# TritonDataCenter/registrar

Hardware: NVIDIA H100
Metric: service-records/sec (higher is better)
Workload: dtype u8

## Files before the change

### registrar_b200/csrc/regk_api.cu

```cuda
#include <cuda_runtime.h>

#include <algorithm>
#include <cstdarg>
#include <cstdio>
#include <cstdlib>
#include <cstring>
#include <map>
#include <mutex>
#include <string>
#include <vector>

#include "../../include/regk.h"
#include "regk_kernels.cuh"
#include "regk_gather.cuh"
#include "regk_peersync.cuh"
#include "regk_service.cuh"
#include "regk_jute.cuh"
#include "regk_decode.cuh"
#include "regk_parents.cuh"
#include "regk_skip.cuh"
#include "regk_mkdirp.cuh"
#include "regk_types.hpp"

using namespace regk;

namespace {

thread_local std::string g_create_error;

struct DevBuf {
    void *p = nullptr;
    size_t cap = 0;
};

struct HostBuf {
    void *p = nullptr;
    size_t cap = 0;
};

}

struct regk_ctx {
    int device = 0;
    cudaStream_t own_stream = nullptr;
    cudaStream_t stream = nullptr;
    std::string err;
    int sm_count = 0;
    int max_smem_optin = 0;

    std::vector<std::string> types;
    std::vector<uint8_t> blob_host;
    DevBuf blob_dev;
    uint32_t max_type_q = 0;

    DevBuf in[11];
    DevBuf path_bytes, path_off, json_bytes, json_off, off32_p, off32_j;
    HostBuf h_path_bytes, h_path_off, h_json_bytes, h_json_off, h_running;
    cudaStream_t s_h2d = nullptr, s_d2h = nullptr;
    struct HostSet {
        DevBuf in[11];
        DevBuf path_bytes, path_off, json_bytes, json_off, off32_p, off32_j;
        HostBuf h_path_bytes, h_path_off, h_json_bytes, h_json_off;
        cudaEvent_t e_in = nullptr, e_out = nullptr;
    };
    HostSet hset[2];
    uint64_t hseq = 0;
    uint32_t *h_gather_flag = nullptr;
    double json_mean_seen = 0.0;
    uint64_t json_est_seen = 0;
    bool json_learning = true;
    regk_job job{};
    bool job_bound = false;
    unsigned long long job_seq = 0;
    DevBuf job_bases;
    unsigned long long *h_job_bases = nullptr;
    const uint8_t *last_path_bytes = nullptr;
    const unsigned long long *last_path_off = nullptr;
    uint64_t last_n = 0;
    const uint8_t *last_json_bytes = nullptr;
    const unsigned long long *last_json_off = nullptr;
    uint64_t last_json_n = 0;
    DevBuf jute_bytes, jute_off;
    HostBuf h_jute_bytes, h_jute_off;
    DevBuf dec_in[4], dec_rec, dec_dom, dec_ports;
    HostBuf h_dec_rec, h_dec_dom, h_dec_ports;
    const uint32_t *last_host_off = nullptr;
    uint32_t last_host_stride = 0;
    bool last_alias = false;
    DevBuf svc_in[7], svc_work;
    DevBuf par_len, par_slot, par_table, par_totals, par_unique;
    cudaEvent_t par_ev[2] = {nullptr, nullptr};
    HostBuf h_par_len, h_par_unique, h_par_count;
    enum { MK_PLEN, MK_PSLOT, MK_PTABLE, MK_PTOTALS, MK_PUNIQUE, MK_FLAGS, MK_LIST0, MK_LIST1, MK_TOTALS, MK_TABLE,
           MK_COUNT, MK_DREC, MK_DLEN, MK_DBYTES, MK_DOFF, MK_DEPTH, MK_INVALID, MK_ZERO, MK_FBYTES, MK_FOFF, MK_NBUF };
    DevBuf mk[MK_NBUF];
    HostBuf h_mk_count, h_mk_drec, h_mk_dlen, h_mk_dbytes, h_mk_doff, h_mk_depth, h_mk_invalid, h_mk_fbytes, h_mk_foff;
    cudaEvent_t mk_ev[4] = {nullptr, nullptr, nullptr, nullptr};
    bool mk_valid = false;
    uint64_t mk_n_dirs = 0, mk_bytes = 0;
    std::vector<cudaEvent_t> pipe_events;
    DevBuf skip_work, skip_in[11], skip_off_p, skip_off_j, skip_index, skip_bits;
    HostBuf h_skip_status, h_skip_index, h_skip_bits;
    struct SkipLast {
        bool valid = false;
        uint64_t n = 0, n_skipped = 0;
        uint32_t bad_bits = 0;
    } skip_last;
    DevBuf work;
    static constexpr int NWORK = 4;
    DevBuf work_ring[NWORK];
    cudaEvent_t ws_clean[NWORK] = {nullptr, nullptr, nullptr, nullptr};
    size_t ws_clean_bytes[NWORK] = {0, 0, 0, 0};
    cudaStream_t s_side = nullptr;
    uint64_t ws_seq = 0;

    struct Slot {
        cudaEvent_t ev[6] = {nullptr, nullptr, nullptr, nullptr, nullptr, nullptr};
        PathParams path_params{};
        size_t path_smem = 0;
        bool path_alias = false, did_path = false;
        DevStatus *d_status = nullptr;
        DevStatus *h_status = nullptr;
        int ring = -1;
        int hset = -1;
        bool d2h_issued = false;
        bool timed = true;
        const uint8_t *dev_path_bytes = nullptr;
        const unsigned long long *dev_path_off = nullptr;
        const uint8_t *dev_json_bytes = nullptr;
        const unsigned long long *dev_json_off = nullptr;
        const uint32_t *dev_host_off = nullptr;
// ... 23 lines not shown
namespace {

int fail(regk_ctx *c, int code, const char *fmt, ...)
{
    char buf[512];
    va_list ap;
    va_start(ap, fmt);
    vsnprintf(buf, sizeof buf, fmt, ap);
    va_end(ap);
    if (c)
        c->err = buf;
    else
        g_create_error = buf;
    return code;
}

#define CK(call)                                                                                   \
    do {                                                                                           \
        cudaError_t e_ = (call);                                                                   \
        if (e_ != cudaSuccess)                                                                     \
            return fail(ctx, REGK_ERR_CUDA, "%s failed: %s (%s:%d)", #call, cudaGetErrorString(e_), \
                __FILE__, __LINE__);                                                               \
    } while (0)

int ensure_dev(regk_ctx *ctx, DevBuf &b, size_t bytes)
{
    bytes = (bytes + 255) & ~(size_t)255;
    if (bytes <= b.cap)
        return REGK_OK;
    if (b.p)
        CK(cudaFree(b.p));
    b.p = nullptr;
    b.cap = 0;
    size_t want = bytes + bytes / 8;
    cudaError_t e = cudaMalloc(&b.p, want);
    if (e != cudaSuccess) {
        cudaGetLastError();
        e = cudaMalloc(&b.p, bytes);
        want = bytes;
    }
    if (e != cudaSuccess)
        return fail(ctx, REGK_ERR_NOMEM, "cudaMalloc(%zu) failed: %s", bytes, cudaGetErrorString(e));
    b.cap = want;
    return REGK_OK;
}

int ensure_host(regk_ctx *ctx, HostBuf &b, size_t bytes)
{
    bytes = (bytes + 4095) & ~(size_t)4095;
    if (bytes <= b.cap)
        return REGK_OK;
    if (b.p)
        CK(cudaFreeHost(b.p));
    b.p = nullptr;
    b.cap = 0;
    cudaError_t e = cudaMallocHost(&b.p, bytes);
    if (e != cudaSuccess)
        return fail(ctx, REGK_ERR_NOMEM, "cudaMallocHost(%zu) failed: %s", bytes, cudaGetErrorString(e));
    b.cap = bytes;
    return REGK_OK;
}

int64_t opt_get(const regk_ctx *c, const char *name, int64_t dflt)
{
    auto it = c->opt.find(name);
    return it == c->opt.end() ? dflt : it->second;
}

size_t align16(size_t v)
{
    return (v + 15) & ~(size_t)15;
}

bool smem_attr_needs_raise(int device, int which, size_t bytes)
{
    static std::mutex mu;
    static size_t high[64][4];
    std::lock_guard<std::mutex> lock(mu);
    size_t &h = high[device & 63][which];
    if (bytes <= h)
        return false;
    h = bytes;
    return true;
}

}

__global__ void __launch_bounds__(256) regk_off32_kernel(const unsigned long long *__restrict__ src, uint32_t *__restrict__ dst, uint64_t n1)
{
    const uint64_t i = (uint64_t)blockIdx.x * 256 + threadIdx.x;
    if (i < n1)
        dst[i] = (uint32_t)src[i];
}

static int narrow_offsets(regk_ctx *ctx, const void *src64, DevBuf &dst32, uint64_t n, cudaStream_t s)
{
    int rc = ensure_dev(ctx, dst32, (n + 1) * 4);
    if (rc)
        return rc;
    regk_off32_kernel<<<(unsigned)((n + 1 + 255) / 256), 256, 0, s>>>((const unsigned long long *)src64, (uint32_t *)dst32.p, n + 1);
    CK(cudaGetLastError());
    return REGK_OK;
}

struct HostPipe {
    uint64_t chunk = 0, nchunks = 0, nsuper_chunk = 0;
    unsigned long long *running = nullptr;
    uint64_t path_cap = 0, json_cap = 0;
    const void *src[11] = {};
    void *dev[11] = {};
};

static bool chunk_bounds_ok(const regk_batch *b, uint64_t chunk, bool do_path, bool do_json, bool alias)
{
    const uint64_t n = b->n;
    auto ok = [&](const uint32_t *off) {
        if (!off)
            return true;
        uint32_t prev = off[0];
        const uint32_t last = off[n];
        if (prev != 0 && prev > last)
            return false;
        for (uint64_t r = chunk; r < n; r += chunk) {
            if (off[r] < prev || off[r] > last)
                return false;
            prev = off[r];
        }
        return true;
    };
    return (!do_path || (ok(b->domain_off) && (alias || ok(b->host_off)))) &&
           (!do_json || (ok(b->addr_off) && ok(b->ports_off)));
}

static int run_pipelined(regk_ctx *ctx, const regk_batch *b, regk_result *res, const PathParams &pp0, size_t path_smem,
    const JsonParams &jp0, size_t json_smem, const HostPipe &hp)
{
    const uint64_t n = b->n;
    const bool alias = b->flags & REGK_NODE_ALIAS;
    const bool do_path = !(b->flags & REGK_NO_PATH), do_json = !(b->flags & REGK_NO_JSON);
    const uint32_t stride = b->host_stride;
    cudaStream_t s = ctx->stream;
    int rc;
    if (!ctx->s_h2d) {
        CK(cudaStreamCreateWithFlags(&ctx->s_h2d, cudaStreamNonBlocking));
        CK(cudaStreamCreateWithFlags(&ctx->s_d2h, cudaStreamNonBlocking));
    }
    while (ctx->pipe_events.size() < 3 * hp.nchunks + 2) {
        cudaEvent_t e;
        CK(cudaEventCreateWithFlags(&e, cudaEventDisableTiming));
        ctx->pipe_events.push_back(e);
    }
    if ((rc = ensure_host(ctx, ctx->h_path_bytes, hp.path_cap)) || (rc = ensure_host(ctx, ctx->h_path_off, (n + 1) * 8)) ||
        (rc = ensure_host(ctx, ctx->h_json_bytes, hp.json_cap)) || (rc = ensure_host(ctx, ctx->h_json_off, (n + 1) * 8)) ||
        (rc = ensure_host(ctx, ctx->h_running, (hp.nchunks + 2) * 8)))
        return rc;
    unsigned long long *h_running = (unsigned long long *)ctx->h_running.p;
    DevStatus *d_status = pp0.status ? pp0.status : jp0.status;
    DevStatus *h_status = ctx->slots[0].h_status;

    cudaEvent_t e_ready = ctx->pipe_events[3 * hp.nchunks];
    CK(cudaEventRecord(e_ready, s));
    CK(cudaStreamWaitEvent(ctx->s_h2d, e_ready, 0));

    const uint32_t *dom_off = (const uint32_t *)b->domain_off, *host_off = (const uint32_t *)b->host_off,
                   *addr_off = (const uint32_t *)b->addr_off, *ports_off = (const uint32_t *)b->ports_off;
    auto h2d = [&](int i, size_t byte_lo, size_t byte_hi) -> cudaError_t {
// ... 560 lines not shown
    CK(cudaSetDevice(ctx->device));
    std::vector<std::string> raw(ntypes);
    for (uint32_t i = 0; i < ntypes; i++)
        raw[i].assign(types[i], lens ? lens[i] : strlen(types[i]));
    std::vector<uint8_t> blob;
    uint32_t maxq = 0;
    std::string why;
    const int brc = build_type_blob(raw, &blob, &maxq, &why);
    if (brc)
        return fail(ctx, brc == 1 ? REGK_ERR_OUT_OF_DOMAIN : REGK_ERR_INVALID_ARG, "regk_set_types: %s", why.c_str());
    int rc = ensure_dev(ctx, ctx->blob_dev, blob.size());
    if (rc)
        return rc;
    CK(cudaMemcpyAsync(ctx->blob_dev.p, blob.data(), blob.size(), cudaMemcpyHostToDevice, ctx->stream));
    CK(cudaStreamSynchronize(ctx->stream));
    ctx->types = raw;
    ctx->blob_host = blob;
    ctx->max_type_q = maxq;
    ctx->json_mean_seen = 0.0;
    ctx->json_learning = true;
    return REGK_OK;
}

void *regk_host_alloc(regk_ctx *ctx, size_t bytes)
{
    if (!ctx)
        return nullptr;
    void *p = nullptr;
    cudaSetDevice(ctx->device);
    if (cudaMallocHost(&p, bytes ? bytes : 1) != cudaSuccess) {
        cudaGetLastError();
        return nullptr;
    }
    return p;
}

void regk_host_free(regk_ctx *ctx, void *p)
{
    (void)ctx;
    if (p)
        cudaFreeHost(p);
}

void *regk_dev_alloc(regk_ctx *ctx, size_t bytes)
{
    if (!ctx)
        return nullptr;
    void *p = nullptr;
    cudaSetDevice(ctx->device);
    if (cudaMalloc(&p, bytes ? bytes : 1) != cudaSuccess) {
        cudaGetLastError();
        return nullptr;
    }
    return p;
}

void regk_dev_free(regk_ctx *ctx, void *p)
{
    (void)ctx;
    if (p)
        cudaFree(p);
}

int regk_memcpy_h2d(regk_ctx *ctx, void *dst_dev, const void *src_host, size_t bytes)
{
    if (!ctx)
        return REGK_ERR_INVALID_ARG;
    CK(cudaSetDevice(ctx->device));
    CK(cudaMemcpyAsync(dst_dev, src_host, bytes, cudaMemcpyHostToDevice, ctx->stream));
    CK(cudaStreamSynchronize(ctx->stream));
    return REGK_OK;
}

int regk_memcpy_d2h(regk_ctx *ctx, void *dst_host, const void *src_dev, size_t bytes)
{
    if (!ctx)
        return REGK_ERR_INVALID_ARG;
    CK(cudaSetDevice(ctx->device));
    CK(cudaMemcpyAsync(dst_host, src_dev, bytes, cudaMemcpyDeviceToHost, ctx->stream));
    CK(cudaStreamSynchronize(ctx->stream));
    return REGK_OK;
}

int regk_sync(regk_ctx *ctx)
{
    if (!ctx)
        return REGK_ERR_INVALID_ARG;
    CK(cudaSetDevice(ctx->device));
    CK(cudaStreamSynchronize(ctx->stream));
    if (ctx->h_gather_flag && *ctx->h_gather_flag) {
        *ctx->h_gather_flag = 0;
        return fail(ctx, REGK_ERR_INVALID_ARG, "regk_gather_push: the totals table exceeds the whole-job buffers or disagrees with the shard; nothing was stored");
    }
    return REGK_OK;
}

int regk_ipc_export(regk_ctx *ctx, const void *dev_ptr, unsigned char handle[REGK_IPC_HANDLE_BYTES])
{
    if (!ctx || !dev_ptr || !handle)
        return fail(ctx, REGK_ERR_INVALID_ARG, "regk_ipc_export: NULL argument");
    static_assert(sizeof(cudaIpcMemHandle_t) == REGK_IPC_HANDLE_BYTES, "IPC handle size");
    CK(cudaSetDevice(ctx->device));
    cudaIpcMemHandle_t h;
    CK(cudaIpcGetMemHandle(&h, const_cast<void *>(dev_ptr)));
    memcpy(handle, &h, sizeof h);
    return REGK_OK;
}

int regk_ipc_open(regk_ctx *ctx, const unsigned char handle[REGK_IPC_HANDLE_BYTES], void **peer_ptr)
{
    if (!ctx || !handle || !peer_ptr)
        return fail(ctx, REGK_ERR_INVALID_ARG, "regk_ipc_open: NULL argument");
    CK(cudaSetDevice(ctx->device));
    cudaIpcMemHandle_t h;
    memcpy(&h, handle, sizeof h);
    *peer_ptr = nullptr;
    CK(cudaIpcOpenMemHandle(peer_ptr, h, cudaIpcMemLazyEnablePeerAccess));
    return REGK_OK;
}

int regk_ipc_close(regk_ctx *ctx, void *peer_ptr)
{
    if (!ctx || !peer_ptr)
        return REGK_ERR_INVALID_ARG;
    CK(cudaSetDevice(ctx->device));
    CK(cudaIpcCloseMemHandle(peer_ptr));
    return REGK_OK;
}

int regk_gather_push(regk_ctx *ctx, const regk_result *shard, const regk_gather *g)
{
    if (!ctx || !shard || !g)
        return fail(ctx, REGK_ERR_INVALID_ARG, "regk_gather_push: NULL argument");
    if (g->world == 0 || g->world > REGK_MAX_PEERS || g->rank >= g->world)
        return fail(ctx, REGK_ERR_INVALID_ARG, "regk_gather_push: world %u / rank %u out of range (at most %d peers)",
            g->world, g->rank, REGK_MAX_PEERS);
    if (!(shard->flags & REGK_OUT_DEVICE) || !shard->path_off || !shard->json_off)
        return fail(ctx, REGK_ERR_INVALID_ARG, "regk_gather_push: the shard must be a finished REGK_OUT_DEVICE result");
    if (!g->totals || g->rec_base + shard->n > g->n_total)
        return fail(ctx, REGK_ERR_INVALID_ARG, "regk_gather_push: totals missing or record range outside the job");
    for (uint32_t q = 0; q < g->world; q++)
        if (!g->path_bytes[q] || !g->path_off[q] || !g->json_bytes[q] || !g->json_off[q] ||
            (((uintptr_t)g->path_bytes[q] | (uintptr_t)g->json_bytes[q]) & 15) || (((uintptr_t)g->path_off[q] | (uintptr_t)g->json_off[q]) & 7))
            return fail(ctx, REGK_ERR_INVALID_ARG, "regk_gather_push: buffer of rank %u missing or misaligned", q);
    CK(cudaSetDevice(ctx->device));
    if (!ctx->h_gather_flag) {
        CK(cudaMallocHost((void **)&ctx->h_gather_flag, sizeof(uint32_t)));
        *ctx->h_gather_flag = 0;
    }
    GatherParams p{};
    p.world = g->world;
    p.rank = g->rank;
    p.n_local = shard->n;
    p.rec_base = g->rec_base;
    p.n_total = g->n_total;
    p.totals = (const unsigned long long *)g->totals;
    p.src_path = shard->path_bytes;
    p.src_json = shard->json_bytes;
    p.src_path_off = (const unsigned long long *)shard->path_off;
    p.src_json_off = (const unsigned long long *)shard->json_off;
    for (uint32_t q = 0; q < g->world; q++) {
        p.dst_path[q] = (uint8_t *)g->path_bytes[q];
        p.dst_json[q] = (uint8_t *)g->json_bytes[q];
        p.dst_path_off[q] = (unsigned long long *)g->path_off[q];
        p.dst_json_off[q] = (unsigned long long *)g->json_off[q];
    }
// ... 230 lines not shown
        wk = (uint8_t *)ctx->work.p;
        CK(cudaMemsetAsync(wk, 0, work_bytes, s));
    } else {
        ring = (int)(ctx->ws_seq++ % regk_ctx::NWORK);
        if (!ctx->s_side) {
            CK(cudaStreamCreateWithFlags(&ctx->s_side, cudaStreamNonBlocking));
            for (auto &e : ctx->ws_clean)
                CK(cudaEventCreateWithFlags(&e, cudaEventDisableTiming));
        }
        const size_t cap_before = ctx->work_ring[ring].cap;
        if ((rc = ensure_dev(ctx, ctx->work_ring[ring], work_bytes)))
            return rc;
        if (ctx->work_ring[ring].cap != cap_before)
            ctx->ws_clean_bytes[ring] = 0;
        wk = (uint8_t *)ctx->work_ring[ring].p;
        if (ctx->ws_clean_bytes[ring] >= work_bytes)
        {
            if (cudaEventQuery(ctx->ws_clean[ring]) != cudaSuccess) {
                cudaGetLastError();
                CK(cudaStreamWaitEvent(s, ctx->ws_clean[ring], 0));
            }
        }
        else
            CK(cudaMemsetAsync(wk, 0, work_bytes, s));
    }
    DevStatus *d_status = (DevStatus *)wk;

    if (n == 0 && !job) {
        CK(cudaMemsetAsync(o_path_off.p, 0, 8, s));
        CK(cudaMemsetAsync(o_json_off.p, 0, 8, s));
    }
    const uint32_t force_generic = (uint32_t)opt_get(ctx, "force_generic", 0);

    PathParams pp{};
    size_t path_smem = 0;
    if (n && do_path) {
        pp.n = n;
        pp.domain_bytes = (const uint8_t *)dev[0];
        pp.domain_off = (const uint32_t *)dev[1];
        pp.host_bytes = (const uint8_t *)dev[2];
        pp.host_off = (const uint32_t *)dev[3];
        pp.host_stride = b->host_stride;
        pp.out_bytes = out_path_bytes;
        pp.out_off = out_path_off;
        pp.out_capacity = out_path_cap;
        if (job) {
            pp.bias_in = d_bases;
            fill_peers(pp.peer, J, J.path_bytes, J.path_off);
        }
        pp.exact = 0;
        pp.tile_total = (uint32_t *)(wk + totals_p_off);
        pp.super_total = (unsigned long long *)(wk + super_p_off);
        pp.status = d_status;
        pp.dom_limit = dom_len;
        pp.host_limit = host_len;
        pp.force_generic = force_generic;
        const uint64_t mean_dom_tile = std::min<uint64_t>(dom_len, dom_len * TILE / std::max<uint64_t>(n, 1)) + 1;
        uint32_t dom_cap = (uint32_t)opt_get(ctx, "dom_cap", 0);
        if (!dom_cap)
            dom_cap = (uint32_t)std::min<uint64_t>(std::max<uint64_t>(align16(mean_dom_tile * 5 / 4 + 384), 2048), 49152);
        dom_cap = (uint32_t)((dom_cap + 127) & ~127u);
        uint32_t host_cap = 0;
        if (!alias) {
            const uint64_t mean_host_tile = pp.host_off ? std::min<uint64_t>(host_len, host_len * TILE / std::max<uint64_t>(n, 1)) + 1
                                                        : (uint64_t)TILE * b->host_stride;
            host_cap = (uint32_t)std::min<uint64_t>(align16((pp.host_off ? mean_host_tile * 3 / 2 + 512 : mean_host_tile) + 16), 49152);
        }
        const uint32_t out_cap = (uint32_t)align16((uint64_t)dom_cap + host_cap + 2 * TILE + 32);
        path_smem = 16 + (size_t)dom_cap + 32 + dom_cap / 8 + 16 + (alias ? 0 : host_cap + 32) + out_cap + 32;
        if (path_smem > (size_t)ctx->max_smem_optin)
            return fail(ctx, REGK_ERR_INVALID_ARG, "path kernel needs %zu B of shared memory (> %d)", path_smem, ctx->max_smem_optin);
        pp.dom_cap = dom_cap;
        pp.host_cap = host_cap;
        pp.out_cap = out_cap;
        if (smem_attr_needs_raise(ctx->device, alias ? 0 : 1, path_smem)) {
            if (alias) {
                CK(cudaFuncSetAttribute(regk_path_kernel<true, false>, cudaFuncAttributeMaxDynamicSharedMemorySize, (int)path_smem));
                CK(cudaFuncSetAttribute(regk_path_kernel<true, true>, cudaFuncAttributeMaxDynamicSharedMemorySize, (int)path_smem));
            } else {
                CK(cudaFuncSetAttribute(regk_path_kernel<false, false>, cudaFuncAttributeMaxDynamicSharedMemorySize, (int)path_smem));
                CK(cudaFuncSetAttribute(regk_path_kernel<false, true>, cudaFuncAttributeMaxDynamicSharedMemorySize, (int)path_smem));
            }
        }
    }
    JsonParams jp{};
    size_t json_smem = 0;
    if (n && do_json) {
        jp.n = n;
        jp.type_id = (const uint8_t *)dev[4];
        jp.addr_bytes = (const uint8_t *)dev[5];
        jp.addr_off = (const uint32_t *)dev[6];
        jp.ttl = (const int32_t *)dev[7];
        jp.ports_off = (const uint32_t *)dev[8];
        jp.ports = (const uint32_t *)dev[9];
        jp.ports_present = (const uint8_t *)dev[10];
        jp.frag_blob = (const uint8_t *)ctx->blob_dev.p;
        jp.ntypes = (uint32_t)ctx->types.size();
        jp.blob_bytes = (uint32_t)ctx->blob_host.size();
        jp.out_bytes = out_json_bytes;
        jp.out_off = out_json_off;
        jp.out_capacity = out_json_cap;
        if (job) {
            jp.base_in = d_bases + 4;
            fill_peers(jp.peer, J, J.json_bytes, J.json_off);
        }
        jp.tile_total = (uint32_t *)(wk + totals_j_off);
        jp.super_total = (unsigned long long *)(wk + super_j_off);
        jp.status = d_status;
        jp.addr_limit = addr_len;
        jp.ports_limit = ports_len;
        jp.force_generic = force_generic;
        uint32_t out_cap = (uint32_t)opt_get(ctx, "json_out_cap", 0);
        if (!out_cap) {
            uint64_t mean = 42 + 2ull * ctx->max_type_q + (n ? 2 * addr_len / n : 0) + 11 +
                (ports_len ? 11 + (n ? 6 * ports_len / n : 0) : 0) + 2;
            uint64_t tile_bytes = mean * TILE * 9 / 8 + 512;
            slot.json_est = mean;
            slot.json_learned = false;
            if (ctx->json_mean_seen > 0.0 && n >= 4096 && ctx->json_est_seen == mean) {
                const uint64_t seen = (uint64_t)(ctx->json_mean_seen + 1.0);
                if (seen < mean) {
                    tile_bytes = seen * TILE * 17 / 16 + 1024;
                    slot.json_learned = true;
                }
            }
            out_cap = (uint32_t)std::min<uint64_t>(align16(tile_bytes), 98304);
        }
        out_cap = (uint32_t)align16(out_cap);
        jp.out_cap = out_cap;
        json_smem = (size_t)jp.blob_bytes + out_cap + 32;
        if (json_smem > (size_t)ctx->max_smem_optin)
            return fail(ctx, REGK_ERR_INVALID_ARG, "json kernel needs %zu B of shared memory (> %d)", json_smem, ctx->max_smem_optin);
        if (smem_attr_needs_raise(ctx->device, 2, json_smem)) {
            CK(cudaFuncSetAttribute(regk_json_kernel, cudaFuncAttributeMaxDynamicSharedMemorySize, (int)json_smem));
        }
    }

    if (pipelined) {
        HostPipe hp;
        hp.chunk = chunk_records;
        hp.nchunks = nchunks;
        hp.nsuper_chunk = nsuper_chunk;
        hp.running = (unsigned long long *)(wk + running_off);
        hp.path_cap = path_cap;
        hp.json_cap = json_cap;
        for (int i = 0; i < 11; i++) {
            hp.src[i] = src[i];
            hp.dev[i] = need[i] && src[i] ? ctx->in[i].p : nullptr;
        }
        rc = run_pipelined(ctx, b, res, pp, path_smem, jp, json_smem, hp);
        ctx->skip_last = regk_ctx::SkipLast{};
        if (rc == REGK_ERR_OUT_OF_DOMAIN && (b->flags & REGK_SKIP_BAD) && !(res->bad_bits & REGK_BAD_TOO_LARGE)) {
            slot.n = n;
            slot.flags = b->flags;
            slot.hset = -1;
            slot.off32 = false;
            slot.timed = false;
            slot.launches = res->launches;
            for (int i = 0; i < 11; i++)
                slot.dev_in[i] = dev[i];
            slot.in_len[0] = dom_len, slot.in_len[1] = host_len, slot.in_len[2] = addr_len, slot.in_len[3] = ports_len;
            slot.in_stride = b->host_stride;
            DevStatus st{};
            st.bad_bits = res->bad_bits;
            st.first_bad = ~(unsigned long long)res->first_bad;
            return finish_skip(ctx, &slot, st, res);
        }
        if (rc == REGK_OK && (b->flags & REGK_SKIP_BAD)) {
            ctx->skip_last.valid = true;
            ctx->skip_last.n = n;
        }
        if (rc == REGK_OK) {
            ctx->last_path_bytes = do_path ? pp.out_bytes : nullptr;
            ctx->last_path_off = do_path ? pp.out_off : nullptr;
            ctx->last_n = do_path ? n : 0;
            ctx->last_json_bytes = do_json ? jp.out_bytes : nullptr;
            ctx->last_json_off = do_json ? jp.out_off : nullptr;
            ctx->last_json_n = do_json ? n : 0;
            ctx->last_host_off = pp.host_off;
            ctx->last_host_stride = pp.host_stride;
            ctx->last_alias = alias;
        }
        if (rc != REGK_ERR_STATE + 100)
            return rc;
        for (int i = 0; i < 11; i++)
            if (dev[i] && sz[i])
                CK(cudaMemcpyAsync(ctx->in[i].p, src[i], sz[i], cudaMemcpyHostToDevice, s));
        CK(cudaMemsetAsync(wk, 0, work_bytes, s));
    }

    uint32_t launches = 0;
    slot.did_path = false;
    slot.d_status = d_status;
    slot.dev_path_bytes = (n && do_path && !job) ? pp.out_bytes : nullptr;
    slot.dev_path_off = (n && do_path && !job) ? pp.out_off : nullptr;
    slot.dev_json_bytes = (n && do_json && !job) ? jp.out_bytes : nullptr;
    slot.dev_json_off = (n && do_json && !job) ? jp.out_off : nullptr;
    slot.dev_host_off = pp.host_off;
    slot.host_stride = pp.host_stride;
    slot.alias = alias;
    const bool fused_len = n && do_path && do_json;
    const int64_t time_every = std::max<int64_t>(1, opt_get(ctx, "time_every", 1));
    const bool timed = ctx->seq % (uint64_t)time_every == 0;
    slot.timed = timed;
    if (job) {
        const uint64_t my_paths = dom_len + host_len + (alias ? 1 : 2) * n;
        if ((rc = launch_exchange(ctx, my_paths, n, nullptr, 0, d_bases, (unsigned long long *)J.path_off[J.rank] + J.n_total)))
            return rc;
        launches++;
    }
    if (timed)
        CK(cudaEventRecord(slot.ev[0], s));
    if (n && do_path) {
        if (alias)
            regk_path_kernel<true, false><<<(unsigned)ntiles, TILE, path_smem, s>>>(pp, fused_len ? jp : JsonParams{});
        else
            regk_path_kernel<false, false><<<(unsigned)ntiles, TILE, path_smem, s>>>(pp, fused_len ? jp : JsonParams{});
        CK(cudaGetLastError());
// ... 1132 lines not shown
```

### registrar_b200/csrc/regk_kernels.cuh

```cuda
#ifndef REGK_KERNELS_CUH
#define REGK_KERNELS_CUH

#include <cuda_runtime.h>
#include <stdint.h>

#include "../../include/regk.h"
#include "regk_core.cuh"

namespace regk {

#ifndef REGK_TILE
#define REGK_TILE 128
#endif
#ifndef REGK_MINB_PATH
#define REGK_MINB_PATH 8
#endif
#ifndef REGK_MINB_JSON
#define REGK_MINB_JSON 10
#endif
constexpr int TILE = REGK_TILE;
constexpr int WARPS = TILE / 32;

struct DevStatus {
    uint32_t bad_bits;
// ... 147 lines not shown
__device__ __forceinline__ void bulk_s2g(uint8_t *gdst, const uint8_t *smem_src, uint32_t bytes)
{
    asm volatile("cp.async.bulk.global.shared::cta.bulk_group [%0], [%1], %2;"
                 ::"l"(gdst), "r"(smem_u32(smem_src)), "r"(bytes) : "memory");
}

__device__ __forceinline__ void flush_out_job(uint8_t *gout, uint8_t *const *s_pb, uint32_t npeers, const uint8_t *smem,
    uint64_t gbase, uint32_t total)
{
    if (threadIdx.x != 0 || total == 0)
        return;
    const uint64_t a0 = gbase & ~15ull;
    const uint32_t lo = (uint32_t)(gbase - a0);
    const uint32_t hi = lo + total;
    const uint32_t b_first = lo >> 4, b_last = (hi - 1u) >> 4;
    for (uint32_t d = 0; d <= npeers; d++) {
        uint8_t *g = (d == 0 ? gout : s_pb[d - 1]) + a0;
        if (b_first == b_last) {
            store_block_part(g + 16u * b_first, smem + 16u * b_first, lo & 15u, ((hi - 1u) & 15u) + 1u);
        } else {
            uint32_t body_lo = lo, body_hi = hi;
            if (lo & 15u) {
                store_block_part(g + 16u * b_first, smem + 16u * b_first, lo & 15u, 16u);
                body_lo = 16u * (b_first + 1u);
            }
            if (hi & 15u) {
                store_block_part(g + 16u * b_last, smem + 16u * b_last, 0u, hi & 15u);
                body_hi = 16u * b_last;
            }
            if (body_hi > body_lo)
                bulk_s2g(g + body_lo, smem + body_lo, body_hi - body_lo);
        }
    }
    asm volatile("cp.async.bulk.commit_group;" ::: "memory");
    asm volatile("cp.async.bulk.wait_group.read 0;" ::: "memory");
}

__device__ __forceinline__ void copy_range_to_peers(const uint8_t *gown, uint8_t *const *s_pb, uint32_t npeers, uint64_t gbase,
    uint32_t total)
{
    const uint64_t end = gbase + total;
    uint64_t body_lo = (gbase + 15ull) & ~15ull, body_hi = end & ~15ull;
    if (body_hi <= body_lo)
        body_lo = body_hi = end;
    for (uint64_t b = body_lo + 16ull * threadIdx.x; b < body_hi; b += 16ull * TILE) {
        const uint4 v = *reinterpret_cast<const uint4 *>(gown + b);
        for (uint32_t q = 0; q < npeers; q++)
            stg_v4(s_pb[q] + b, v);
    }
    for (uint64_t i = gbase + threadIdx.x; i < body_lo; i += TILE)
        for (uint32_t q = 0; q < npeers; q++)
            s_pb[q][i] = gown[i];
    for (uint64_t i = body_hi + threadIdx.x; i < end; i += TILE)
        for (uint32_t q = 0; q < npeers; q++)
            s_pb[q][i] = gown[i];
}

template <typename T>
__device__ __forceinline__ T block_scan(T *warp_sum , T v, T *total)
{
    const uint32_t lane = threadIdx.x & 31u, warp = threadIdx.x >> 5;
    T incl = v;
    #pragma unroll
    for (int d = 1; d < 32; d <<= 1) {
        T up = __shfl_up_sync(0xFFFFFFFFu, incl, d);
        if (lane >= (uint32_t)d)
            incl += up;
    }
    __syncthreads();
    if (lane == 31)
        warp_sum[warp] = incl;
    __syncthreads();
    T before = 0, tot = 0;
    #pragma unroll
    for (int w = 0; w < WARPS; w++) {
        T s = warp_sum[w];
        if ((uint32_t)w < warp)
            before += s;
        tot += s;
    }
    *total = tot;
    return before + incl - v;
}

constexpr uint32_t SUPER = 64;

__device__ __forceinline__ void add_tile_total(uint32_t *tile_total, unsigned long long *super_total, uint32_t tile,
    uint32_t warp_bytes)
{
    if (warp_bytes) {
        atomicAdd(tile_total + tile, warp_bytes);
        atomicAdd(super_total + tile / SUPER, (unsigned long long)warp_bytes);
    }
}

__device__ __forceinline__ unsigned long long tile_base_from_totals(const uint32_t *tile_total,
    const unsigned long long *super_total, uint32_t tile)
{
    const uint32_t lane = threadIdx.x & 31u;
    const uint32_t nsuper = tile / SUPER;
    unsigned long long acc = 0;
    for (uint32_t i = lane; i < nsuper; i += 32)
        acc += super_total[i];
    for (uint32_t i = nsuper * SUPER + lane; i < tile; i += 32)
        acc += tile_total[i];
    #pragma unroll
    for (int d = 16; d > 0; d >>= 1)
        acc += __shfl_xor_sync(0xFFFFFFFFu, acc, d);
    return acc;
}

__device__ __forceinline__ void report_bad(DevStatus *st, uint32_t bad, uint64_t rec)
{
    if (bad) {
        atomicOr(&st->bad_bits, bad);
        atomicMax(&st->first_bad, ~(unsigned long long)rec);
    }
}


struct JsonParams {
    uint64_t n;
    const uint8_t *type_id;
    const uint8_t *addr_bytes;
    const uint32_t *addr_off;
    const int32_t *ttl;
    const uint32_t *ports_off;
    const uint32_t *ports;
    const uint8_t *ports_present;
    const uint8_t *frag_blob;
    uint32_t ntypes;
    uint32_t blob_bytes;
    uint8_t *out_bytes;
    unsigned long long *out_off;
    uint64_t out_capacity;
    uint64_t rec0;
    const unsigned long long *base_in;
    unsigned long long *base_out;
    uint32_t *tile_total;
    unsigned long long *super_total;
    DevStatus *status;
    uint64_t addr_limit, ports_limit;
    uint32_t out_cap;
    uint32_t force_generic;
    PeerDst peer;
};

struct JsonMeta {
    uint32_t tid, a0, al, p0, k;
    int32_t ttl;
    bool has_ttl, has_ports;
    uint32_t bad;
};

__device__ __forceinline__ JsonMeta json_meta(const JsonParams &p, uint64_t r)
{
    JsonMeta m;
    m.bad = 0;
    m.tid = p.type_id[r];
    if (m.tid >= p.ntypes) {
        m.bad |= BAD_TYPE_ID;
        m.tid = 0;
    }
    m.a0 = p.addr_off[r];
    uint32_t a1 = p.addr_off[r + 1];
    if (a1 < m.a0 || a1 > p.addr_limit) {
        m.bad |= BAD_TOO_LARGE;
        a1 = m.a0 = 0;
    }
    m.al = a1 - m.a0;
    if (m.al == 0)
        m.bad |= BAD_ADDR_BYTE;
    m.ttl = p.ttl ? p.ttl[r] : INT32_MIN;
    m.has_ttl = m.ttl != INT32_MIN;
    m.p0 = 0;
    m.k = 0;
    if (p.ports_off) {
        m.p0 = p.ports_off[r];
        uint32_t p1 = p.ports_off[r + 1];
        if (p1 < m.p0 || p1 > p.ports_limit) {
            m.bad |= BAD_TOO_LARGE;
            p1 = m.p0 = 0;
        }
        m.k = p1 - m.p0;
    }
    m.has_ports = p.ports_present ? (p.ports_present[r] != 0) : (m.k > 0);
    if (!m.has_ports)
        m.k = 0;
    return m;
}

__device__ __forceinline__ uint32_t json_meta_len(const JsonParams &p, const JsonMeta &m, const TypeFrag &tf)
{
    const uint32_t *pp = p.ports + m.p0;
    const uint32_t k = m.k;
    uint32_t port_digits = 0;
    if (k) {
        const uint32_t v0 = pp[0], v1 = k > 1u ? pp[1] : 0u, v2 = k > 2u ? pp[2] : 0u, v3 = k > 3u ? pp[3] : 0u;
        port_digits = ndigits_u32(v0) + (k > 1u ? ndigits_u32(v1) : 0u) + (k > 2u ? ndigits_u32(v2) : 0u) +
                      (k > 3u ? ndigits_u32(v3) : 0u);
        for (uint32_t i = 4; i < k; i++)
            port_digits += ndigits_u32(pp[i]);
    }
    return json_length(tf.f1_len, tf.f2_len, m.al, m.has_ttl, m.ttl, m.has_ports, m.k, port_digits);
}


struct PathParams {
    uint64_t n;
    const uint8_t *domain_bytes;
    const uint32_t *domain_off;
    const uint8_t *host_bytes;
    const uint32_t *host_off;
    uint32_t host_stride;
    uint8_t *out_bytes;
    unsigned long long *out_off;
    uint64_t out_capacity;
    uint64_t rec0;
    uint64_t off_bias;
    uint32_t exact;
    uint32_t *tile_total;
    unsigned long long *super_total;
    DevStatus *status;
    uint64_t dom_limit, host_limit;
    uint32_t dom_cap, host_cap, out_cap;
    uint32_t force_generic;
    const unsigned long long *bias_in;
    PeerDst peer;
};

template <bool ALIAS>
__device__ __forceinline__ unsigned long long path_cf(const PathParams &p, uint64_t r)
{
    unsigned long long v = (unsigned long long)p.domain_off[r];
    if (ALIAS)
        return v + r;
    return v + 2ull * r + (p.host_off ? (unsigned long long)p.host_off[r] : r * (unsigned long long)p.host_stride);
}

template <bool ALIAS>
__global__ void __launch_bounds__(TILE) regk_path_len_kernel(const PathParams p)
{
    const uint32_t tile = blockIdx.x, t = threadIdx.x;
    const uint64_t r0 = (uint64_t)tile * TILE;
    const uint32_t nrec = (uint32_t)min((uint64_t)TILE, p.n - r0);
    uint32_t len = 0;
    if (t < nrec) {
        const uint64_t r = r0 + t;
        const uint32_t d0 = p.domain_off[r], d1 = p.domain_off[r + 1];
        const uint32_t L = (d1 >= d0 && d1 <= p.dom_limit) ? d1 - d0 : 0;
        uint32_t H = 0;
        if (!ALIAS) {
            if (p.host_off) {
                const uint32_t a = p.host_off[r], b = p.host_off[r + 1];
                H = b >= a ? b - a : 0;
            } else {
                H = p.host_stride;
            }
        }
        const GuardedWords dsrc{reinterpret_cast<const uint32_t *>(p.domain_bytes)};
        len = path_length(scan_domain(dsrc, d0, L), L, H, ALIAS);
    }
    #pragma unroll
    for (int d = 16; d > 0; d >>= 1)
        len += __shfl_xor_sync(0xFFFFFFFFu, len, d);
    if ((t & 31u) == 0)
        add_tile_total(p.tile_total, p.super_total, tile, len);
}

__device__ __forceinline__ void payload_length_side_job(const JsonParams &jp, const JsonMeta &jm, const TypeFrag &jtf,
    bool live, uint32_t tile)
{
    uint32_t jl = live ? json_meta_len(jp, jm, jtf) : 0;
    #pragma unroll
    for (int d = 16; d > 0; d >>= 1)
        jl += __shfl_xor_sync(0xFFFFFFFFu, jl, d);
    if ((threadIdx.x & 31u) == 0)
        add_tile_total(jp.tile_total, jp.super_total, tile, jl);
}

struct TilePlan {
    unsigned long long tile_base;
    unsigned long long HB0;
    uint32_t D0, D1, HA1;
    uint32_t nd, nh;
    uint32_t host_span;
    uint32_t tile_total;
    uint32_t flags;
};
enum : uint32_t { PLAN_BROKEN = 1, PLAN_FITS = 2, PLAN_BULK = 4, PLAN_ROOM = 8 };

template <bool ALIAS, bool EXACT>
__global__ void __launch_bounds__(TILE, REGK_MINB_PATH) regk_path_kernel(const PathParams p, const JsonParams jp)
{
    extern __shared__ __align__(16) uint8_t smem[];
    __shared__ uint32_t warp_sum[WARPS];
    __shared__ __align__(8) uint64_t s_bar;
    __shared__ TilePlan s_plan;
    __shared__ uint8_t *s_pb[REGK_MAX_PEERS - 1];
    __shared__ unsigned long long *s_po[REGK_MAX_PEERS - 1];
    const uint32_t npeers = p.peer.n;
    if (npeers)
        peer_tables(p.peer, s_pb, s_po);
    uint8_t *s_dom = smem + 16;
    uint8_t *s_bits = s_dom + p.dom_cap + 32;
    uint8_t *s_host = s_bits + p.dom_cap / 8 + 16;
    uint8_t *s_out = s_host + (ALIAS ? 0 : p.host_cap + 32);

    const uint32_t tile = blockIdx.x;
    const uint32_t t = threadIdx.x;
    const uint64_t r0 = (uint64_t)tile * TILE;
    const uint32_t nrec = (uint32_t)min((uint64_t)TILE, p.n - r0);
    const bool live = t < nrec;
    const uint32_t tl = live ? t : 0u;
    const uint64_t r = r0 + tl;
    constexpr bool exact = EXACT;
    const bool var_host = !ALIAS && p.host_off != nullptr;
    const uint32_t per_rec = ALIAS ? 1u : 2u;

    if (t == 0) {
        mbar_init(&s_bar, 1);
        TilePlan q;
        q.D0 = p.domain_off[r0];
        q.D1 = p.domain_off[r0 + nrec];
        unsigned long long HB1 = 0;
        q.HB0 = 0;
        q.HA1 = 0;
        if (var_host) {
            q.HB0 = p.host_off[r0];
            q.HA1 = p.host_off[r0 + nrec];
            HB1 = q.HA1;
        } else if (!ALIAS) {
            q.HB0 = r0 * p.host_stride;
            HB1 = q.HB0 + (unsigned long long)nrec * p.host_stride;
        }
        const bool broken = q.D1 < q.D0 || q.D1 > p.dom_limit || (!ALIAS && (HB1 < q.HB0 || HB1 > p.host_limit));
        const uint32_t dom_span = q.D1 - q.D0, host_span = (uint32_t)(HB1 - q.HB0);
        const uint32_t dom_lead = q.D0 & 15u, host_lead = (uint32_t)q.HB0 & 15u;
        q.nd = (dom_lead + dom_span + 15u) & ~15u;
        q.nh = ALIAS ? 0u : (host_lead + host_span + 15u) & ~15u;
        const bool fits = !broken && !p.force_generic && dom_lead + dom_span <= p.dom_cap &&
            (ALIAS || host_lead + host_span <= p.host_cap) && dom_span + host_span + 2u * nrec + 16u <= p.out_cap;
        const bool bulk = fits && (unsigned long long)(q.D0 & ~15u) + q.nd <= p.dom_limit &&
            (ALIAS || (q.HB0 & ~15ull) + q.nh <= p.host_limit);
        if (bulk) {
            mbar_expect_tx(&s_bar, q.nd + q.nh);
            if (q.nd)
                bulk_g2s(s_dom, p.domain_bytes + (q.D0 & ~15u), q.nd, &s_bar);
            if (q.nh)
                bulk_g2s(s_host, p.host_bytes + (q.HB0 & ~15ull), q.nh, &s_bar);
        }
        q.tile_base = (unsigned long long)q.D0 + q.HB0 + (unsigned long long)per_rec * r0 + p.off_bias +
            (p.bias_in ? *p.bias_in : 0ull);
        q.tile_total = dom_span + host_span + per_rec * nrec;
        q.host_span = host_span;
        q.flags = (broken ? PLAN_BROKEN : 0u) | (fits ? PLAN_FITS : 0u) | (bulk ? PLAN_BULK : 0u);
        if (!exact && !broken && q.tile_base + q.tile_total <= p.out_capacity)
            q.flags |= PLAN_ROOM;
        s_plan = q;
    }

    const uint32_t d0 = p.domain_off[r], d1 = p.domain_off[r + 1];
    uint32_t ha = 0, hb = 0;
    if (var_host) {
        ha = p.host_off[r];
        hb = p.host_off[r + 1];
    }
    const bool side = !EXACT && jp.n != 0;
    JsonMeta jm;
    TypeFrag jtf;
    if (side) {
        jm = json_meta(jp, r);
        jtf = reinterpret_cast<const TypeFrag *>(jp.frag_blob)[jm.tid];
    }
    unsigned long long exact_base = 0;
    if (exact && t < 32)
        exact_base = tile_base_from_totals(p.tile_total, p.super_total, tile);
    if (exact && t == 0)
        *reinterpret_cast<unsigned long long *>(warp_sum) = exact_base;
    __syncthreads();

    if (side)
        payload_length_side_job(jp, jm, jtf, live, tile);

    const uint32_t flags = s_plan.flags;
    const uint32_t D0 = s_plan.D0;
    unsigned long long tile_base = s_plan.tile_base;
    uint32_t tile_total = s_plan.tile_total;
    bool room = flags & PLAN_ROOM;
    if (exact) {
        tile_base = *reinterpret_cast<const unsigned long long *>(warp_sum) + p.off_bias + (p.bias_in ? *p.bias_in : 0ull);
        tile_total = p.tile_total[tile];
        room = !(flags & PLAN_BROKEN) && tile_base + tile_total <= p.out_capacity;
        __syncthreads();
    }
    uint32_t bad = 0;
    bool rec_ok = d1 >= d0 && d0 >= D0 && d1 <= s_plan.D1;
    uint32_t hrel, H;
    if (ALIAS) {
        hrel = 0;
        H = 0;
    } else if (var_host) {
        rec_ok = rec_ok && hb >= ha && ha >= (uint32_t)s_plan.HB0 && hb <= s_plan.HA1;
        hrel = ha - (uint32_t)s_plan.HB0;
        H = hb - ha;
    } else {
        hrel = tl * p.host_stride;
        H = p.host_stride;
    }
    uint32_t L = d1 - d0;
    if (!live || !rec_ok) {
        L = 0;
        H = 0;
    }
    if (live && (!rec_ok || (flags & PLAN_BROKEN)))
        bad = BAD_TOO_LARGE;
    uint32_t local = rec_ok ? (d0 - D0) + hrel + per_rec * tl : 0u;
    const uint32_t slot = L + H + per_rec;

    if (flags & PLAN_BROKEN) {
    } else if (flags & PLAN_FITS) {
        const uint32_t nd = s_plan.nd, nh = s_plan.nh;
        if (flags & PLAN_BULK) {
            mbar_wait(&s_bar, 0);
        } else {
            stage_in(s_dom, p.domain_bytes, D0, s_plan.D1, p.dom_limit);
            if (!ALIAS)
                stage_in(s_host, p.host_bytes, s_plan.HB0, s_plan.HB0 + s_plan.host_span, p.host_limit);
            __syncthreads();
        }
        uint32_t *dom_w = reinterpret_cast<uint32_t *>(s_dom);
        const uint32_t *bits_w = reinterpret_cast<const uint32_t *>(s_bits);
        const uint32_t *host_w = reinterpret_cast<const uint32_t *>(s_host);
        uint32_t suspicious = prepass_domain(dom_w, reinterpret_cast<uint16_t *>(s_bits), nd >> 4, t, TILE);
        if (!ALIAS)
            suspicious |= prepass_host(host_w, nh >> 4, t, TILE);
        suspicious = __syncthreads_or(suspicious != 0);
        const uint32_t doff = (D0 & 15u) + (d0 - D0);
        const uint32_t hoff = ((uint32_t)s_plan.HB0 & 15u) + hrel;
        const DomainInfo di = domain_info(bits_w, rec_ok ? doff : 0u, L);
        if (suspicious) {
            bad |= recheck_domain(s_dom, bits_w, doff, L);
            if (!ALIAS && live && rec_ok)
                bad |= check_host(PaddedWords{host_w}, hoff, H);
        } else if (!ALIAS && live && rec_ok && H <= 2) {
            bad |= check_host(PaddedWords{host_w}, hoff, H);
        }
        const uint32_t len = (live && rec_ok) ? path_length2(di, L, H, ALIAS) : 0;
        if (exact) {
            uint32_t tot;
            local = block_scan<uint32_t>(warp_sum, len, &tot);
        } else if (live && len != slot) {
            atomicOr(&p.status->needs_exact, 1u);
        }
        if (live) {
            p.out_off[r] = tile_base + local;
            for (uint32_t q = 0; q < npeers; q++)
                s_po[q][r] = tile_base + local;
        }
        if (room) {
            WordSink sink;
            sink.init(reinterpret_cast<uint32_t *>(s_out), local + ((uint32_t)tile_base & 15u));
            if (live && rec_ok) {
                if (!ALIAS && H >= 24u)
                    emit_path2<ALIAS, true>(dom_w, bits_w, doff, L, di, host_w, hoff, H, sink);
                else
                    emit_path2<ALIAS, false>(dom_w, bits_w, doff, L, di, host_w, hoff, H, sink);
            }
            __syncthreads();
            if (live)
                sink.tail();
            fence_proxy_async();
            __syncthreads();
            if (npeers)
                flush_out_job(p.out_bytes, s_pb, npeers, s_out, tile_base, tile_total);
            else
                flush_out(p.out_bytes, s_out, tile_base, tile_total);
        }
    } else {
        if (t == 0)
            atomicAdd(&p.status->generic_tiles, 1u);
        const unsigned long long HB0 = s_plan.HB0;
        const GuardedWords dsrc{reinterpret_cast<const uint32_t *>(p.domain_bytes)};
        const GuardedWords hsrc{reinterpret_cast<const uint32_t *>(p.host_bytes + (var_host ? 0 : HB0))};
        const uint32_t hoff = var_host ? (uint32_t)HB0 + hrel : hrel;
        const DomainStats st = scan_domain(dsrc, d0, L);
        bad |= st.bad;
        if (!ALIAS && live && rec_ok)
            bad |= check_host(hsrc, hoff, H);
        const uint32_t len = (live && rec_ok) ? path_length(st, L, H, ALIAS) : 0;
        if (exact) {
            uint32_t tot;
            local = block_scan<uint32_t>(warp_sum, len, &tot);
        } else if (live && len != slot) {
            atomicOr(&p.status->needs_exact, 1u);
        }
        if (live) {
            p.out_off[r] = tile_base + local;
            for (uint32_t q = 0; q < npeers; q++)
                s_po[q][r] = tile_base + local;
        }
        if (room && live && rec_ok) {
            ByteSink sink;
            sink.init(p.out_bytes + tile_base + local);
            emit_path<ALIAS>(dsrc, d0, L, hsrc, hoff, H, sink);
        }
        if (npeers && room) {
            __syncthreads();
            copy_range_to_peers(p.out_bytes, s_pb, npeers, tile_base, tile_total);
        }
    }
    if (!room && !(flags & PLAN_BROKEN) && t == 0)
        atomicOr(&p.status->overflow, 1u);
    if (live)
        report_bad(p.status, bad, p.rec0 + r);
    if (r0 + nrec == p.n && t == 0) {
        if (p.peer.job) {
            p.status->path_total = tile_base + tile_total - (p.bias_in ? *p.bias_in : 0ull) - p.off_bias;
        } else {
            p.out_off[p.n] = tile_base + tile_total;
            p.status->path_total = tile_base + tile_total;
        }
    }
}


__global__ void __launch_bounds__(TILE) regk_json_len_kernel(const JsonParams p, uint32_t ntiles)
{
    const uint32_t t = threadIdx.x, lane = t & 31u;
    for (uint32_t tile = blockIdx.x; tile < ntiles; tile += gridDim.x) {
        const uint64_t r = (uint64_t)tile * TILE + t;
        uint32_t len = 0;
        if (r < p.n) {
            const JsonMeta m = json_meta(p, r);
            const TypeFrag tf = reinterpret_cast<const TypeFrag *>(p.frag_blob)[m.tid];
            len = json_meta_len(p, m, tf);
        }
        #pragma unroll
        for (int d = 16; d > 0; d >>= 1)
            len += __shfl_xor_sync(0xFFFFFFFFu, len, d);
        if (lane == 0)
            add_tile_total(p.tile_total, p.super_total, tile, len);
    }
}

struct JsonPlan {
    unsigned long long tile_base;
    uint32_t tile_total;
    uint32_t flags;
};

__global__ void __launch_bounds__(TILE, REGK_MINB_JSON) regk_json_kernel(const JsonParams p)
{
    extern __shared__ __align__(16) uint8_t smem[];
    __shared__ uint32_t warp_sum[WARPS];
    __shared__ __align__(8) uint64_t s_bar;
    __shared__ JsonPlan s_plan;
    __shared__ uint8_t *s_pb[REGK_MAX_PEERS - 1];
    __shared__ unsigned long long *s_po[REGK_MAX_PEERS - 1];
    const uint32_t npeers = p.peer.n;
    if (npeers)
        peer_tables(p.peer, s_pb, s_po);
    uint8_t *s_blob = smem;
    uint8_t *s_out = smem + p.blob_bytes;

    const uint32_t t = threadIdx.x;
    const uint32_t tile = blockIdx.x;
    const uint64_t r0 = (uint64_t)tile * TILE;
    const uint32_t nrec = (uint32_t)min((uint64_t)TILE, p.n - r0);
    const bool live = t < nrec;
    const uint64_t r = r0 + (live ? t : 0);

    if (t < 32) {
        if (t == 0) {
            mbar_init(&s_bar, 1);
            mbar_expect_tx(&s_bar, p.blob_bytes);
            bulk_g2s(s_blob, p.frag_blob, p.blob_bytes, &s_bar);
        }
        const unsigned long long b = tile_base_from_totals(p.tile_total, p.super_total, tile) + (p.base_in ? *p.base_in : 0ull);
        if (t == 0) {
            JsonPlan q;
            q.tile_base = b;
            q.tile_total = p.tile_total[tile];
            q.flags = (b + q.tile_total <= p.out_capacity ? PLAN_ROOM : 0u) |
                (!p.force_generic && q.tile_total + 16u <= p.out_cap ? PLAN_FITS : 0u);
            s_plan = q;
        }
    }

    const JsonMeta m = json_meta(p, r);
    uint32_t bad = m.bad;
    const uint32_t a0 = m.a0, al = m.al, k = m.k;

    const GuardedWords asrc{reinterpret_cast<const uint32_t *>(p.addr_bytes)};
    uint32_t aw[4] = {0, 0, 0, 0};
    {
        const uint32_t n16 = al < 16u ? al : 16u;
        const uint32_t sh = (a0 & 3u) * 8u;
        uint32_t wi = a0 >> 2;
        uint32_t lo = n16 ? asrc.word(wi) : 0u;
        #pragma unroll
        for (int w = 0; w < 4; w++) {
            if (n16 > 4u * w) {
                const uint32_t nb = min(4u, n16 - 4u * w);
                const uint32_t hi = asrc.word_hi(wi + 1, sh + 8u * nb > 32u || n16 > 4u * (w + 1));
                const uint32_t keep = low_bytes(nb);
                aw[w] = funnel_r(lo, hi, sh) & keep;
                if (addr_word_bad(aw[w], keep))
                    bad |= BAD_ADDR_BYTE;
                lo = hi;
                wi++;
            }
        }
        for (uint32_t i = a0 + 16u; i < a0 + al; i++) {
            const uint32_t c = p.addr_bytes[i];
            if (c < 0x20u || c >= 0x80u || c == 0x22u || c == 0x5Cu)
                bad |= BAD_ADDR_BYTE;
        }
    }
    const TypeFrag tf = reinterpret_cast<const TypeFrag *>(p.frag_blob)[m.tid];
    const uint32_t len = live ? json_meta_len(p, m, tf) : 0;
    uint32_t tot;
    const uint32_t local = block_scan<uint32_t>(warp_sum, len, &tot);
    mbar_wait(&s_bar, 0);
    const unsigned long long tile_base = s_plan.tile_base;
    const uint32_t tile_total = s_plan.tile_total;
    const uint32_t flags = s_plan.flags;
    if (live) {
        p.out_off[r] = tile_base + local;
        for (uint32_t q = 0; q < npeers; q++)
            s_po[q][r] = tile_base + local;
    }

    const PaddedWords blob{reinterpret_cast<const uint32_t *>(s_blob)};
    const uint32_t *ports = p.ports + m.p0;
    auto port = [ports](uint32_t i) { return ports[i]; };
    if (!(flags & PLAN_ROOM)) {
        if (t == 0)
            atomicOr(&p.status->overflow, 1u);
    } else if (flags & PLAN_FITS) {
        WordSink sink;
        sink.init(reinterpret_cast<uint32_t *>(s_out), local + ((uint32_t)tile_base & 15u));
        if (live)
            emit_json(blob, tf, aw, asrc, a0, al, m.has_ttl, m.ttl, m.has_ports, k, port, sink);
        __syncthreads();
        if (live)
            sink.tail();
        fence_proxy_async();
        __syncthreads();
        if (npeers)
            flush_out_job(p.out_bytes, s_pb, npeers, s_out, tile_base, tile_total);
        else
            flush_out(p.out_bytes, s_out, tile_base, tile_total);
    } else {
        if (t == 0)
            atomicAdd(&p.status->generic_tiles, 1u);
        if (live) {
            ByteSink sink;
            sink.init(p.out_bytes + tile_base + local);
            emit_json(blob, tf, aw, asrc, a0, al, m.has_ttl, m.ttl, m.has_ports, k, port, sink);
        }
        if (npeers) {
            __syncthreads();
            copy_range_to_peers(p.out_bytes, s_pb, npeers, tile_base, tile_total);
        }
    }
    if (live)
        report_bad(p.status, bad, p.rec0 + r);
    if (r0 + nrec == p.n && t == 0) {
        if (p.peer.job) {
            p.status->json_total = tile_base + tile_total - (p.base_in ? *p.base_in : 0ull);
        } else {
            p.out_off[p.n] = tile_base + tile_total;
            p.status->json_total = tile_base + tile_total;
            if (p.base_out)
                *p.base_out = tile_base + tile_total;
        }
    }
}

}
#endif
```

Baseline: 6.527 billion.

## Prefetch input slices of tiles one half-wave ahead into L2

Each CTA's last warp issues cp.async.bulk.prefetch.L2 for the per-record input arrays (offsets, type ids, ttl, ports) of the tile that sits half a resident wave ahead. The JSON kernel also reads that tile's offset bounds and prefetches the variable-length address and port byte ranges. The lookahead distance comes from a cached occupancy query. The aim is to hide DRAM latency for later tiles, at the cost of extra prefetch instructions, a few dependent loads in one warp, and possible L2 pollution. Optional phase-timestamp instrumentation is added behind a compile flag.

```diff
diff --git a/registrar_b200/csrc/regk_api.cu b/registrar_b200/csrc/regk_api.cu
--- a/registrar_b200/csrc/regk_api.cu
+++ b/registrar_b200/csrc/regk_api.cu
@@ -47,6 +47,7 @@
     std::string err;
     int sm_count = 0;
     int max_smem_optin = 0;
+    std::map<size_t, uint32_t> wave_ctas[3];
 
     std::vector<std::string> types;
     std::vector<uint8_t> blob_host;
@@ -236,6 +237,18 @@
         return false;
     h = bytes;
     return true;
+}
+
+int lookahead_tiles(regk_ctx *ctx, int which, const void *kernel, size_t smem, uint32_t *out)
+{
+    auto it = ctx->wave_ctas[which].find(smem);
+    if (it == ctx->wave_ctas[which].end()) {
+        int per_sm = 0;
+        CK(cudaOccupancyMaxActiveBlocksPerMultiprocessor(&per_sm, kernel, TILE, smem));
+        it = ctx->wave_ctas[which].emplace(smem, (uint32_t)per_sm * (uint32_t)ctx->sm_count).first;
+    }
+    *out = it->second / 2;
+    return REGK_OK;
 }
 
 }
@@ -962,6 +975,21 @@
     return REGK_OK;
 }
 
+#ifdef REGK_PHASE_STAMPS
+int regk_phase_stamps(regk_ctx *ctx, void *dev_buf, uint64_t tiles)
+{
+    if (!ctx)
+        return REGK_ERR_INVALID_ARG;
+    CK(cudaSetDevice(ctx->device));
+    CK(cudaStreamSynchronize(ctx->stream));
+    unsigned long long *p = (unsigned long long *)dev_buf;
+    const unsigned long long cap = dev_buf ? tiles : 0;
+    CK(cudaMemcpyToSymbol(regk::g_phase_buf, &p, sizeof(p)));
+    CK(cudaMemcpyToSymbol(regk::g_phase_cap, &cap, sizeof(cap)));
+    return REGK_OK;
+}
+#endif
+
 int regk_sync(regk_ctx *ctx)
 {
     if (!ctx)
@@ -1358,6 +1386,9 @@
                 CK(cudaFuncSetAttribute(regk_path_kernel<false, true>, cudaFuncAttributeMaxDynamicSharedMemorySize, (int)path_smem));
             }
         }
+        if ((rc = lookahead_tiles(ctx, alias ? 0 : 1, alias ? (const void *)regk_path_kernel<true, false> : (const void *)regk_path_kernel<false, false>,
+                 path_smem, &pp.lookahead)))
+            return rc;
     }
     JsonParams jp{};
     size_t json_smem = 0;
@@ -1410,6 +1441,8 @@
         if (smem_attr_needs_raise(ctx->device, 2, json_smem)) {
             CK(cudaFuncSetAttribute(regk_json_kernel, cudaFuncAttributeMaxDynamicSharedMemorySize, (int)json_smem));
         }
+        if ((rc = lookahead_tiles(ctx, 2, (const void *)regk_json_kernel, json_smem, &jp.lookahead)))
+            return rc;
     }
 
     if (pipelined) {
diff --git a/registrar_b200/csrc/regk_kernels.cuh b/registrar_b200/csrc/regk_kernels.cuh
--- a/registrar_b200/csrc/regk_kernels.cuh
+++ b/registrar_b200/csrc/regk_kernels.cuh
@@ -253,6 +253,45 @@
     *total = tot;
     return before + incl - v;
 }
+
+__device__ __forceinline__ void prefetch_l2(const void *base, uint64_t lo, uint64_t hi, uint64_t limit)
+{
+    hi = min(hi, limit);
+    const uintptr_t a = ((uintptr_t)base + lo + 15u) & ~(uintptr_t)15, b = ((uintptr_t)base + hi) & ~(uintptr_t)15;
+    if (base && hi > lo && b > a)
+        asm volatile("cp.async.bulk.prefetch.L2.global [%0], %1;" ::"l"(a), "r"((uint32_t)(b - a)));
+}
+
+__device__ __forceinline__ void prefetch_slice(const void *a, uint32_t esz, uint64_t r0, uint64_t r1, uint64_t n)
+{
+    prefetch_l2(a, esz * r0, esz * r1, esz * n);
+}
+
+__device__ __forceinline__ void look_tile(uint32_t lookahead, uint64_t n, uint64_t &r0, uint64_t &r1)
+{
+    r0 = ((uint64_t)blockIdx.x + lookahead) * TILE;
+    r1 = min(r0 + TILE, n);
+}
+
+#ifdef REGK_PHASE_STAMPS
+__device__ unsigned long long *g_phase_buf;
+__device__ unsigned long long g_phase_cap;
+__device__ __forceinline__ void phase_stamp(uint32_t kernel, uint32_t phase)
+{
+    if (threadIdx.x == 0 && g_phase_buf && blockIdx.x < g_phase_cap) {
+        unsigned long long *e = g_phase_buf + ((unsigned long long)kernel * g_phase_cap + blockIdx.x) * 8u;
+        e[phase] = clock64();
+        if (phase == 0) {
+            uint32_t sm;
+            asm volatile("mov.u32 %0, %%smid;" : "=r"(sm));
+            e[7] = sm;
+        }
+    }
+}
+#define REGK_PHASE(kernel, phase) phase_stamp(kernel, phase)
+#else
+#define REGK_PHASE(kernel, phase) ((void)0)
+#endif
 
 constexpr uint32_t SUPER = 64;
 
@@ -314,6 +353,7 @@
     uint64_t addr_limit, ports_limit;
     uint32_t out_cap;
     uint32_t force_generic;
+    uint32_t lookahead;
     PeerDst peer;
 };
 
@@ -374,6 +414,35 @@
             port_digits += ndigits_u32(pp[i]);
     }
     return json_length(tf.f1_len, tf.f2_len, m.al, m.has_ttl, m.ttl, m.has_ports, m.k, port_digits);
+}
+
+__device__ __forceinline__ void look_json(const JsonParams &p, uint32_t j, uint64_t r0, uint64_t r1)
+{
+    if (j == 0)
+        prefetch_slice(p.type_id, 1, r0, r1, p.n);
+    else if (j == 1)
+        prefetch_slice(p.addr_off, 4, r0, r1 + 1, p.n + 1);
+    else if (j == 2)
+        prefetch_slice(p.ttl, 4, r0, r1, p.n);
+    else if (j == 3)
+        prefetch_slice(p.ports_off, 4, r0, r1 + 1, p.n + 1);
+    else if (j == 4)
+        prefetch_slice(p.ports_present, 1, r0, r1, p.n);
+}
+
+__device__ __forceinline__ const uint32_t *look_json_bounds(const JsonParams &p, uint32_t j)
+{
+    return j == 5 ? p.addr_off : j == 6 ? p.ports_off : nullptr;
+}
+
+__device__ __forceinline__ void look_json_bytes(const JsonParams &p, uint32_t j, uint32_t b0, uint32_t b1)
+{
+    if (b1 < b0 || b1 - b0 > 4u * p.out_cap)
+        return;
+    if (j == 5)
+        prefetch_l2(p.addr_bytes, b0, b1, p.addr_limit);
+    else if (j == 6)
+        prefetch_l2(p.ports, 4ull * b0, 4ull * b1, 4ull * p.ports_limit);
 }
 
 
@@ -396,9 +465,22 @@
     uint64_t dom_limit, host_limit;
     uint32_t dom_cap, host_cap, out_cap;
     uint32_t force_generic;
+    uint32_t lookahead;
     const unsigned long long *bias_in;
     PeerDst peer;
 };
+
+template <bool ALIAS>
+__device__ __forceinline__ void look_path(const PathParams &p, const JsonParams &jp, bool side, uint32_t lane, uint64_t r0,
+    uint64_t r1)
+{
+    if (lane == 0)
+        prefetch_slice(p.domain_off, 4, r0, r1 + 1, p.n + 1);
+    else if (!ALIAS && lane == 1)
+        prefetch_slice(p.host_off, 4, r0, r1 + 1, p.n + 1);
+    else if (side && lane >= 2)
+        look_json(jp, lane - 2, r0, r1);
+}
 
 template <bool ALIAS>
 __device__ __forceinline__ unsigned long long path_cf(const PathParams &p, uint64_t r)
@@ -470,6 +552,7 @@
     __shared__ TilePlan s_plan;
     __shared__ uint8_t *s_pb[REGK_MAX_PEERS - 1];
     __shared__ unsigned long long *s_po[REGK_MAX_PEERS - 1];
+    REGK_PHASE(0, 0);
     const uint32_t npeers = p.peer.n;
     if (npeers)
         peer_tables(p.peer, s_pb, s_po);
@@ -549,7 +632,13 @@
         exact_base = tile_base_from_totals(p.tile_total, p.super_total, tile);
     if (exact && t == 0)
         *reinterpret_cast<unsigned long long *>(warp_sum) = exact_base;
+    if (p.lookahead && tile + p.lookahead < gridDim.x && t >= TILE - 32) {
+        uint64_t l0, l1;
+        look_tile(p.lookahead, p.n, l0, l1);
+        look_path<ALIAS>(p, jp, side, t & 31u, l0, l1);
+    }
     __syncthreads();
+    REGK_PHASE(0, 1);
 
     if (side)
         payload_length_side_job(jp, jm, jtf, live, tile);
@@ -600,6 +689,7 @@
                 stage_in(s_host, p.host_bytes, s_plan.HB0, s_plan.HB0 + s_plan.host_span, p.host_limit);
             __syncthreads();
         }
+        REGK_PHASE(0, 2);
         uint32_t *dom_w = reinterpret_cast<uint32_t *>(s_dom);
         const uint32_t *bits_w = reinterpret_cast<const uint32_t *>(s_bits);
         const uint32_t *host_w = reinterpret_cast<const uint32_t *>(s_host);
@@ -643,10 +733,12 @@
                 sink.tail();
             fence_proxy_async();
             __syncthreads();
+            REGK_PHASE(0, 3);
             if (npeers)
                 flush_out_job(p.out_bytes, s_pb, npeers, s_out, tile_base, tile_total);
             else
                 flush_out(p.out_bytes, s_out, tile_base, tile_total);
+            REGK_PHASE(0, 4);
         }
     } else {
         if (t == 0)
@@ -729,6 +821,7 @@
     __shared__ JsonPlan s_plan;
     __shared__ uint8_t *s_pb[REGK_MAX_PEERS - 1];
     __shared__ unsigned long long *s_po[REGK_MAX_PEERS - 1];
+    REGK_PHASE(1, 0);
     const uint32_t npeers = p.peer.n;
     if (npeers)
         peer_tables(p.peer, s_pb, s_po);
@@ -759,6 +852,17 @@
         }
     }
 
+    const bool look = p.lookahead && tile + p.lookahead < gridDim.x && t >= TILE - 32;
+    uint32_t lb0 = 0, lb1 = 0;
+    if (look) {
+        uint64_t l0, l1;
+        look_tile(p.lookahead, p.n, l0, l1);
+        look_json(p, t & 31u, l0, l1);
+        if (const uint32_t *bo = look_json_bounds(p, t & 31u)) {
+            lb0 = bo[l0];
+            lb1 = bo[l1];
+        }
+    }
     const JsonMeta m = json_meta(p, r);
     uint32_t bad = m.bad;
     const uint32_t a0 = m.a0, al = m.al, k = m.k;
@@ -791,9 +895,13 @@
     }
     const TypeFrag tf = reinterpret_cast<const TypeFrag *>(p.frag_blob)[m.tid];
     const uint32_t len = live ? json_meta_len(p, m, tf) : 0;
+    if (look)
+        look_json_bytes(p, t & 31u, lb0, lb1);
+    REGK_PHASE(1, 1);
     uint32_t tot;
     const uint32_t local = block_scan<uint32_t>(warp_sum, len, &tot);
     mbar_wait(&s_bar, 0);
+    REGK_PHASE(1, 2);
     const unsigned long long tile_base = s_plan.tile_base;
     const uint32_t tile_total = s_plan.tile_total;
     const uint32_t flags = s_plan.flags;
@@ -819,10 +927,12 @@
             sink.tail();
         fence_proxy_async();
         __syncthreads();
+        REGK_PHASE(1, 3);
         if (npeers)
             flush_out_job(p.out_bytes, s_pb, npeers, s_out, tile_base, tile_total);
         else
             flush_out(p.out_bytes, s_out, tile_base, tile_total);
+        REGK_PHASE(1, 4);
     } else {
         if (t == 0)
             atomicAdd(&p.status->generic_tiles, 1u);
```

After: 7.131 billion, median of 6. 1.09x the previous value.
